# musyoku/chainer-speech-recognition

Measured on AMD Instinct MI355X. Metric: utterances/sec (T=1000, 40x3 feat, |V|~3000) CTC train step, higher is better.
Workload: dtype bf16

## Files before the change

### chainer-speech-recognition_amd/csrc/common.hpp

```cpp
#pragma once
#include <hip/hip_runtime.h>
#include <stdint.h>
#include <stddef.h>
#include <stdlib.h>
#include <string.h>

#define ASR_OK 0
#define ASR_ERR_BAD_ARG (-1)
#define ASR_ERR_WORKSPACE (-2)
#define ASR_ERR_UNSUPPORTED (-3)
#define ASR_ERR_LAUNCH (-4)

#define ASR_LAUNCH_CHECK()                                   \
    do {                                                     \
        if (hipGetLastError() != hipSuccess) return ASR_ERR_LAUNCH; \
    } while (0)

namespace asr {

constexpr int kWave = 64;

__device__ __forceinline__ float wave_sum(float v) {
#pragma unroll
    for (int o = 32; o > 0; o >>= 1) v += __shfl_xor(v, o, 64);
// ... 4 lines not shown
    for (int o = 32; o > 0; o >>= 1) v = fmaxf(v, __shfl_xor(v, o, 64));
    return v;
}
__device__ __forceinline__ double wave_sum_d(double v) {
#pragma unroll
    for (int o = 32; o > 0; o >>= 1) v += __shfl_xor(v, o, 64);
    return v;
}

__device__ __forceinline__ float block_sum(float v, float* scratch) {
    const int lane = threadIdx.x & 63, wid = threadIdx.x >> 6, nw = blockDim.x >> 6;
    v = wave_sum(v);
    if (lane == 0) scratch[wid] = v;
    __syncthreads();
    float r = 0.f;
    for (int i = 0; i < nw; ++i) r += scratch[i];
    __syncthreads();
    return r;
}
__device__ __forceinline__ float block_max(float v, float* scratch) {
    const int lane = threadIdx.x & 63, wid = threadIdx.x >> 6, nw = blockDim.x >> 6;
    v = wave_max(v);
    if (lane == 0) scratch[wid] = v;
    __syncthreads();
    float r = scratch[0];
    for (int i = 1; i < nw; ++i) r = fmaxf(r, scratch[i]);
    __syncthreads();
    return r;
}

#ifdef ASR_ACT_F16
#define ASR_ACT_IS_F16 1
__device__ __forceinline__ float bf16_to_f32(uint16_t h) {
    _Float16 v;
    __builtin_memcpy(&v, &h, 2);
    return (float)v;
}
__device__ __forceinline__ uint16_t f32_to_bf16(float f) {
    const _Float16 v = (_Float16)f;
    uint16_t h;
    __builtin_memcpy(&h, &v, 2);
    return h;
}
__device__ __forceinline__ uint32_t pack_bf16x2(float lo, float hi) {
    typedef _Float16 f16x2_t __attribute__((ext_vector_type(2)));
    typedef float f32x2_t __attribute__((ext_vector_type(2)));
    const f32x2_t v = {lo, hi};
    const f16x2_t r = __builtin_convertvector(v, f16x2_t);
    return *reinterpret_cast<const uint32_t*>(&r);
}
#define ASR_MFMA_16x16x32(a, b, c)                                                                                  \
    __builtin_amdgcn_mfma_f32_16x16x32_f16(__builtin_bit_cast(__attribute__((ext_vector_type(8))) _Float16, (a)),   \
                                           __builtin_bit_cast(__attribute__((ext_vector_type(8))) _Float16, (b)), (c), 0, 0, 0)
#else
#define ASR_ACT_IS_F16 0
__device__ __forceinline__ float bf16_to_f32(uint16_t h) { return __uint_as_float(((uint32_t)h) << 16); }
__device__ __forceinline__ uint16_t f32_to_bf16(float f) {
    __bf16 b = (__bf16)f;
    return *reinterpret_cast<uint16_t*>(&b);
}

__device__ __forceinline__ uint32_t pack_bf16x2(float lo, float hi) {
    typedef __bf16 bf16x2_t __attribute__((ext_vector_type(2)));
    typedef float f32x2_t __attribute__((ext_vector_type(2)));
    const f32x2_t v = {lo, hi};
    const bf16x2_t r = __builtin_convertvector(v, bf16x2_t);
    return *reinterpret_cast<const uint32_t*>(&r);
}
#define ASR_MFMA_16x16x32(a, b, c) __builtin_amdgcn_mfma_f32_16x16x32_bf16((a), (b), (c), 0, 0, 0)
#endif

static inline int debug_flag(const char* key, int dflt) {
    const char* e = getenv("ASR_DEBUG");
    if (!e) return dflt;
    const size_t n = strlen(key);
    for (const char* p = e; *p;) {
        while (*p == ',' || *p == ' ') ++p;
        if (strncmp(p, key, n) == 0 && p[n] == '=') return atoi(p + n + 1);
        while (*p && *p != ',') ++p;
    }
    return dflt;
}

static inline size_t align_up(size_t x, size_t a) { return (x + a - 1) / a * a; }
static inline int cdiv(long long a, long long b) { return (int)((a + b - 1) / b); }

}
```

### chainer-speech-recognition_amd/csrc/elementwise.hip

```cpp
#include "common.hpp"
#include "../../include/asr_hip.h"

namespace asr {
namespace ew {

constexpr int kThreads = 256;
static inline int grid_for(long long n) {
    long long g = (n + kThreads - 1) / kThreads;
    if (g > 256 * 16) g = 256 * 16;
    if (g < 1) g = 1;
    return (int)g;
}

__global__ void cast_bf16_kernel(const float* __restrict__ src, uint16_t* __restrict__ dst, long long n) {
    for (long long i = blockIdx.x * (long long)blockDim.x + threadIdx.x; i < n; i += (long long)gridDim.x * blockDim.x)
        dst[i] = f32_to_bf16(src[i]);
}
__global__ void cast_bf16_vec8_kernel(const float4* __restrict__ src, uint4* __restrict__ dst, long long n8) {
    for (long long i = blockIdx.x * (long long)blockDim.x + threadIdx.x; i < n8; i += (long long)gridDim.x * blockDim.x) {
        const float4 a = src[2 * i], b = src[2 * i + 1];
        uint4 o;
        o.x = (uint32_t)f32_to_bf16(a.x) | ((uint32_t)f32_to_bf16(a.y) << 16);
        o.y = (uint32_t)f32_to_bf16(a.z) | ((uint32_t)f32_to_bf16(a.w) << 16);
        o.z = (uint32_t)f32_to_bf16(b.x) | ((uint32_t)f32_to_bf16(b.y) << 16);
        o.w = (uint32_t)f32_to_bf16(b.z) | ((uint32_t)f32_to_bf16(b.w) << 16);
        dst[i] = o;
    }
}
__global__ void transpose_cast_kernel(const float* __restrict__ src, uint16_t* __restrict__ dst, int rows, int cols) {
    __shared__ float tile[32][33];
    const int r0 = blockIdx.y * 32, c0 = blockIdx.x * 32;
    const int tx = threadIdx.x & 31, ty = threadIdx.x >> 5;
    for (int i = ty; i < 32; i += 8) {
        const int r = r0 + i, c = c0 + tx;
        tile[i][tx] = (r < rows && c < cols) ? src[(size_t)r * cols + c] : 0.f;
    }
    __syncthreads();
    for (int i = ty; i < 32; i += 8) {
        const int c = c0 + i, r = r0 + tx;
        if (c < cols && r < rows) dst[(size_t)c * rows + r] = f32_to_bf16(tile[tx][i]);
    }
}
__global__ void __launch_bounds__(256) cast_many_kernel(const long long* __restrict__ jobs, int njobs) {
    __shared__ float tile[64][65];
    __shared__ long long first_tile[256];
    int j = 0;
    if (njobs <= 256) {
        if ((int)threadIdx.x < njobs) first_tile[threadIdx.x] = jobs[threadIdx.x * 6 + 5];
        __syncthreads();
        int lo = 0, hi = njobs - 1;
        while (lo < hi) {
            const int mid = (lo + hi + 1) >> 1;
            if (first_tile[mid] <= (long long)blockIdx.x) lo = mid; else hi = mid - 1;
        }
        j = lo;
    } else {
        while (j + 1 < njobs && (long long)blockIdx.x >= jobs[(j + 1) * 6 + 5]) ++j;
    }
    const float* __restrict__ src = (const float*)jobs[j * 6 + 0];
    uint16_t* __restrict__ dst = (uint16_t*)jobs[j * 6 + 1];
    const int rows = (int)jobs[j * 6 + 2], cols = (int)jobs[j * 6 + 3];
    const bool transpose = jobs[j * 6 + 4] != 0;
    const int local = (int)((long long)blockIdx.x - jobs[j * 6 + 5]);
    const int tiles_c = (cols + 63) / 64;
    const int r0 = (local / tiles_c) * 64, c0 = (local % tiles_c) * 64;
    const int tx = threadIdx.x & 15, ty = threadIdx.x >> 4;
    const bool vec = (cols & 3) == 0;
    if (!transpose) {
        for (int i = ty; i < 64; i += 16) {
            const int r = r0 + i, c = c0 + tx * 4;
            if (r >= rows || c >= cols) continue;
            if (vec) {
                const float4 v = *(const float4*)(src + (size_t)r * cols + c);
                uint2 o;
                o.x = (unsigned)f32_to_bf16(v.x) | ((unsigned)f32_to_bf16(v.y) << 16);
                o.y = (unsigned)f32_to_bf16(v.z) | ((unsigned)f32_to_bf16(v.w) << 16);
                *(uint2*)(dst + (size_t)r * cols + c) = o;
            } else {
                for (int k = 0; k < 4 && c + k < cols; ++k) dst[(size_t)r * cols + c + k] = f32_to_bf16(src[(size_t)r * cols + c + k]);
            }
        }
        return;
    }
    for (int i = ty; i < 64; i += 16) {
        const int r = r0 + i, c = c0 + tx * 4;
        if (vec && r < rows && c < cols) {
            const float4 v = *(const float4*)(src + (size_t)r * cols + c);
            tile[i][tx * 4 + 0] = v.x; tile[i][tx * 4 + 1] = v.y; tile[i][tx * 4 + 2] = v.z; tile[i][tx * 4 + 3] = v.w;
        } else {
            for (int k = 0; k < 4; ++k) tile[i][tx * 4 + k] = (r < rows && c + k < cols) ? src[(size_t)r * cols + c + k] : 0.f;
        }
    }
    __syncthreads();
    const bool vecr = (rows & 3) == 0;
    for (int i = ty; i < 64; i += 16) {
        const int c = c0 + i, r = r0 + tx * 4;
        if (c >= cols || r >= rows) continue;
        if (vecr) {
            uint2 o;
            o.x = (unsigned)f32_to_bf16(tile[tx * 4 + 0][i]) | ((unsigned)f32_to_bf16(tile[tx * 4 + 1][i]) << 16);
            o.y = (unsigned)f32_to_bf16(tile[tx * 4 + 2][i]) | ((unsigned)f32_to_bf16(tile[tx * 4 + 3][i]) << 16);
            *(uint2*)(dst + (size_t)c * rows + r) = o;
        } else {
            for (int k = 0; k < 4 && r + k < rows; ++k) dst[(size_t)c * rows + r + k] = f32_to_bf16(tile[tx * 4 + k][i]);
        }
    }
}
__global__ void bf16_to_f32_kernel(const uint16_t* __restrict__ src, float* __restrict__ dst, long long n) {
    for (long long i = blockIdx.x * (long long)blockDim.x + threadIdx.x; i < n; i += (long long)gridDim.x * blockDim.x)
        dst[i] = bf16_to_f32(src[i]);
}

template <typename SrcT, typename DstT>
__global__ void permute4_kernel(const SrcT* __restrict__ src, DstT* __restrict__ dst, int d0, int d1, int d2, int d3,
                                long long s0, long long s1, long long s2, long long s3) {
    const long long n = (long long)d0 * d1 * d2 * d3;
    for (long long i = blockIdx.x * (long long)blockDim.x + threadIdx.x; i < n; i += (long long)gridDim.x * blockDim.x) {
        long long r = i;
        const int i3 = r % d3; r /= d3;
        const int i2 = r % d2; r /= d2;
        const int i1 = r % d1; r /= d1;
        const int i0 = (int)r;
        const SrcT v = src[i0 * s0 + i1 * s1 + i2 * s2 + i3 * s3];
        float f;
        if (sizeof(SrcT) == 2) f = bf16_to_f32((uint16_t)v); else f = (float)v;
        if (sizeof(DstT) == 2) dst[i] = (DstT)f32_to_bf16(f); else dst[i] = (DstT)f;
    }
}

template <typename SrcT>
__global__ void pack_input_pad_kernel(const SrcT* __restrict__ x, long long sT, long long sB, long long sH, long long sC, int T,
                                      int B, int H, int C, int Cpad, uint16_t* __restrict__ out) {
    const long long n = (long long)T * B * H * Cpad;
    for (long long i = blockIdx.x * (long long)blockDim.x + threadIdx.x; i < n; i += (long long)gridDim.x * blockDim.x) {
        long long r = i;
        const int c = (int)(r % Cpad); r /= Cpad;
        const int h = (int)(r % H); r /= H;
        const int b = (int)(r % B);
        const int t = (int)(r / B);
        uint16_t v = 0;
        if (c < C) {
            const SrcT s = x[t * sT + b * sB + h * sH + c * sC];
            if (sizeof(SrcT) == 2) v = (uint16_t)s; else v = f32_to_bf16((float)s);
        }
        out[i] = v;
    }
}

constexpr int PIP = 72;
__global__ __launch_bounds__(256) void pack_input_pad_time_kernel(const float* __restrict__ x, long long sB, long long sH, long long sC,
                                                                 int T, int B, int H, int C, uint16_t* __restrict__ out) {
    __shared__ __attribute__((aligned(16))) uint16_t tile[64 * PIP];
    const int t0 = blockIdx.x * 64, b = blockIdx.y, h0 = blockIdx.z * 8;
    const int tl = threadIdx.x & 63, rg = threadIdx.x >> 6;
    for (int i = threadIdx.x; i < 64 * PIP / 2; i += 256) reinterpret_cast<uint32_t*>(tile)[i] = 0u;
    __syncthreads();
    for (int rr = rg; rr < C * 8; rr += 4) {
        const int c = rr >> 3, hh = rr & 7;
        if (h0 + hh < H && t0 + tl < T)
            tile[tl * PIP + hh * 8 + c] = f32_to_bf16(x[(long long)(t0 + tl) + b * sB + (h0 + hh) * sH + c * sC]);
    }
    __syncthreads();
#pragma unroll
    for (int k = 0; k < 2; ++k) {
        const int p = threadIdx.x + 256 * k, t = p >> 3, hh = p & 7;
        if (t0 + t < T && h0 + hh < H)
            *reinterpret_cast<uint4*>(out + (((long long)(t0 + t) * B + b) * H + h0 + hh) * 8) = *reinterpret_cast<const uint4*>(tile + t * PIP + hh * 8);
    }
}

template <typename SrcT>
__global__ void im2col_kernel(const SrcT* __restrict__ x, long long sT, long long sB, long long sH, long long sC, int T,
                              int B, int Hin, int Cin, int KH, int KW, int ph, int pt, int Tout, int Hout, int Kp,
                              uint16_t* __restrict__ col) {
    const long long rows = (long long)Tout * B * Hout;
    const long long n = rows * Kp;
    const int Kreal = KH * KW * Cin;
    for (long long i = blockIdx.x * (long long)blockDim.x + threadIdx.x; i < n; i += (long long)gridDim.x * blockDim.x) {
        const int k = (int)(i % Kp);
        long long row = i / Kp;
        uint16_t out = 0;
        if (k < Kreal) {
            const int ci = k % Cin;
            const int kw = (k / Cin) % KW;
            const int kh = k / (Cin * KW);
            const int ho = (int)(row % Hout); row /= Hout;
            const int b = (int)(row % B);
            const int t = (int)(row / B);
// ... 513 lines not shown
#pragma unroll
            for (int q = 0; q < RU; ++q) add(v[q]);
        }
        for (; r < r1; r += nrl) add(*reinterpret_cast<const uint4*>(x + r * ld + c8 * 8));
    }
    if (rl < nrl)
#pragma unroll
        for (int e = 0; e < 8; ++e) red[rl * cols + c8 * 8 + e] = acc[e];
    __syncthreads();
    for (int c = threadIdx.x; c < cols; c += blockDim.x) {
        float s2 = 0.f;
        for (int q = 0; q < nrl; ++q) s2 += red[q * cols + c];
        atomicAdd(out + c, s2);
    }
}

template <int NC>
__global__ __launch_bounds__(256) void colsum_wide_kernel(const uint16_t* __restrict__ x, long long rows, int cols, int ld,
                                                          float* __restrict__ out) {
    const int n8 = cols >> 3;
    const long long chunk = (rows + gridDim.x - 1) / gridDim.x;
    const long long r0 = blockIdx.x * chunk, r1 = min(rows, r0 + chunk);
    float acc[NC][8];
#pragma unroll
    for (int k = 0; k < NC; ++k)
#pragma unroll
        for (int e = 0; e < 8; ++e) acc[k][e] = 0.f;
    constexpr int RU = 4;
    for (long long r = r0; r < r1; r += RU) {
        uint4 v[RU][NC];
#pragma unroll
        for (int q = 0; q < RU; ++q)
#pragma unroll
            for (int k = 0; k < NC; ++k) {
                const int c8 = threadIdx.x + 256 * k;
                v[q][k] = (c8 < n8 && r + q < r1) ? *reinterpret_cast<const uint4*>(x + (r + q) * ld + c8 * 8) : make_uint4(0, 0, 0, 0);
            }
#pragma unroll
        for (int q = 0; q < RU; ++q)
#pragma unroll
            for (int k = 0; k < NC; ++k) {
                const uint32_t w[4] = {v[q][k].x, v[q][k].y, v[q][k].z, v[q][k].w};
#pragma unroll
                for (int e = 0; e < 4; ++e) {
                    acc[k][2 * e] += bf16_to_f32((uint16_t)(w[e] & 0xffff));
                    acc[k][2 * e + 1] += bf16_to_f32((uint16_t)(w[e] >> 16));
                }
            }
    }
#pragma unroll
    for (int k = 0; k < NC; ++k) {
        const int c8 = threadIdx.x + 256 * k;
        if (c8 < n8)
#pragma unroll
            for (int e = 0; e < 8; ++e) atomicAdd(out + c8 * 8 + e, acc[k][e]);
    }
}

}
}

using namespace asr;
using namespace asr::ew;

extern "C" int asr_cast_bf16(void* stream, const float* src, void* dst, int rows, int cols, int transpose) {
    if (!src || !dst || rows <= 0 || cols <= 0) return ASR_ERR_BAD_ARG;
    hipStream_t s = (hipStream_t)stream;
    if (!transpose) {
        const long long n = (long long)rows * cols;
        if ((n & 7) == 0 && ((((uintptr_t)src) | ((uintptr_t)dst)) & 15) == 0)
            hipLaunchKernelGGL(cast_bf16_vec8_kernel, dim3(grid_for(n >> 3)), dim3(kThreads), 0, s, (const float4*)src, (uint4*)dst, n >> 3);
        else
            hipLaunchKernelGGL(cast_bf16_kernel, dim3(grid_for(n)), dim3(kThreads), 0, s, src, (uint16_t*)dst, n);
    } else {
        hipLaunchKernelGGL(transpose_cast_kernel, dim3(cdiv(cols, 32), cdiv(rows, 32)), dim3(256), 0, s, src,
                           (uint16_t*)dst, rows, cols);
    }
    ASR_LAUNCH_CHECK();
    return ASR_OK;
}

extern "C" int asr_cast_bf16_many(void* stream, const long long* jobs_dev, int njobs, long long total_tiles) {
    if (!jobs_dev || njobs <= 0 || total_tiles <= 0 || total_tiles > 0x7fffffffLL) return ASR_ERR_BAD_ARG;
    hipLaunchKernelGGL(cast_many_kernel, dim3((unsigned)total_tiles), dim3(256), 0, (hipStream_t)stream, jobs_dev, njobs);
    ASR_LAUNCH_CHECK();
    return ASR_OK;
}

extern "C" int asr_bf16_to_f32(void* stream, const void* src, float* dst, long long n) {
    if (!src || !dst || n <= 0) return ASR_ERR_BAD_ARG;
    hipLaunchKernelGGL(bf16_to_f32_kernel, dim3(grid_for(n)), dim3(kThreads), 0, (hipStream_t)stream,
                       (const uint16_t*)src, dst, n);
    ASR_LAUNCH_CHECK();
    return ASR_OK;
}

extern "C" int asr_permute4(void* stream, const void* src, int src_bf16, void* dst, int dst_bf16, int d0, int d1, int d2,
                            int d3, long long s0, long long s1, long long s2, long long s3) {
    if (!src || !dst || d0 <= 0 || d1 <= 0 || d2 <= 0 || d3 <= 0) return ASR_ERR_BAD_ARG;
    hipStream_t s = (hipStream_t)stream;
    const long long n = (long long)d0 * d1 * d2 * d3;
    const dim3 g(grid_for(n)), b(kThreads);
    if (src_bf16 && dst_bf16)
        hipLaunchKernelGGL((permute4_kernel<uint16_t, uint16_t>), g, b, 0, s, (const uint16_t*)src, (uint16_t*)dst, d0, d1, d2, d3, s0, s1, s2, s3);
    else if (src_bf16)
        hipLaunchKernelGGL((permute4_kernel<uint16_t, float>), g, b, 0, s, (const uint16_t*)src, (float*)dst, d0, d1, d2, d3, s0, s1, s2, s3);
    else if (dst_bf16)
        hipLaunchKernelGGL((permute4_kernel<float, uint16_t>), g, b, 0, s, (const float*)src, (uint16_t*)dst, d0, d1, d2, d3, s0, s1, s2, s3);
    else
        hipLaunchKernelGGL((permute4_kernel<float, float>), g, b, 0, s, (const float*)src, (float*)dst, d0, d1, d2, d3, s0, s1, s2, s3);
    ASR_LAUNCH_CHECK();
    return ASR_OK;
}

extern "C" int asr_im2col(void* stream, const void* x, int x_bf16, long long sT, long long sB, long long sH, long long sC,
                          int T, int B, int Hin, int Cin, int KH, int KW, int pad_h, int pad_t, int Tout, int Kp,
                          void* col) {
    if (!x || !col || T <= 0 || B <= 0 || Hin <= 0 || Cin <= 0 || KH <= 0 || KW <= 0 || pad_h < 0 || pad_t < 0) return ASR_ERR_BAD_ARG;
    const int Hout = Hin + 2 * pad_h - KH + 1;
    if (Hout <= 0 || Kp < KH * KW * Cin || Tout <= 0 || Tout > T + 2 * pad_t - KW + 1) return ASR_ERR_BAD_ARG;
    const long long n = (long long)Tout * B * Hout * Kp;
    hipStream_t s = (hipStream_t)stream;
    if (x_bf16 && (Cin & 7) == 0 && (Kp & 7) == 0 && sC == 1 && sH == Cin && sB == (long long)Hin * Cin &&
        sT == (long long)B * Hin * Cin && ((((uintptr_t)x) | ((uintptr_t)col)) & 15) == 0 && Kp == KH * KW * Cin) {
        const long long nv = (long long)Tout * B * Hout * KH * KW * (Cin >> 3);
        hipLaunchKernelGGL(im2col_vec8_kernel, dim3(grid_for(nv)), dim3(kThreads), 0, s, (const uint16_t*)x, T, B, Hin, Cin, KH,
                           KW, pad_h, pad_t, Tout, Hout, Kp, (uint16_t*)col);
        ASR_LAUNCH_CHECK();
        return ASR_OK;
    }
    if ((Kp & 7) == 0 && (((uintptr_t)col) & 15) == 0) {
        const long long nc = n >> 3;
        if (x_bf16)
            hipLaunchKernelGGL(im2col_chunk8_kernel<uint16_t>, dim3(grid_for(nc)), dim3(kThreads), 0, s, (const uint16_t*)x, sT, sB, sH,
                               sC, T, B, Hin, Cin, KH, KW, pad_h, pad_t, Tout, Hout, Kp, (uint4*)col);
        else
            hipLaunchKernelGGL(im2col_chunk8_kernel<float>, dim3(grid_for(nc)), dim3(kThreads), 0, s, (const float*)x, sT, sB, sH, sC,
                               T, B, Hin, Cin, KH, KW, pad_h, pad_t, Tout, Hout, Kp, (uint4*)col);
        ASR_LAUNCH_CHECK();
        return ASR_OK;
    }
    if (x_bf16)
        hipLaunchKernelGGL(im2col_kernel<uint16_t>, dim3(grid_for(n)), dim3(kThreads), 0, s, (const uint16_t*)x, sT, sB, sH,
                           sC, T, B, Hin, Cin, KH, KW, pad_h, pad_t, Tout, Hout, Kp, (uint16_t*)col);
    else
        hipLaunchKernelGGL(im2col_kernel<float>, dim3(grid_for(n)), dim3(kThreads), 0, s, (const float*)x, sT, sB, sH, sC,
                           T, B, Hin, Cin, KH, KW, pad_h, pad_t, Tout, Hout, Kp, (uint16_t*)col);
    ASR_LAUNCH_CHECK();
    return ASR_OK;
}

extern "C" int asr_col2im(void* stream, const void* dcol, int T, int B, int Hin, int Cin, int KH, int KW, int pad_h,
                          int pad_t, int Tout, int Kp, void* dx) {
    if (!dcol || !dx || T <= 0 || B <= 0 || Hin <= 0 || Cin <= 0 || pad_h < 0 || pad_t < 0) return ASR_ERR_BAD_ARG;
    const int Hout = Hin + 2 * pad_h - KH + 1;
    if (Hout <= 0 || Kp < KH * KW * Cin || Tout <= 0 || Tout > T + 2 * pad_t - KW + 1) return ASR_ERR_BAD_ARG;
    const long long n = (long long)T * B * Hin * Cin;
    if ((Cin & 7) == 0 && (Kp & 7) == 0 && ((((uintptr_t)dcol) | ((uintptr_t)dx)) & 15) == 0) {
        hipLaunchKernelGGL(col2im_vec8_kernel, dim3(grid_for(n >> 3)), dim3(kThreads), 0, (hipStream_t)stream,
                           (const uint16_t*)dcol, T, B, Hin, Cin, KH, KW, pad_h, pad_t, Tout, Hout, Kp, (uint16_t*)dx);
        ASR_LAUNCH_CHECK();
        return ASR_OK;
    }
    hipLaunchKernelGGL(col2im_kernel, dim3(grid_for(n)), dim3(kThreads), 0, (hipStream_t)stream, (const uint16_t*)dcol, T,
                       B, Hin, Cin, KH, KW, pad_h, pad_t, Tout, Hout, Kp, (uint16_t*)dx);
    ASR_LAUNCH_CHECK();
    return ASR_OK;
// ... 211 lines not shown
```

### chainer-speech-recognition_amd/csrc/layernorm.hip

```cpp
#include "common.hpp"
#include "../../include/asr_hip.h"

namespace asr {
namespace ln {

template <typename T>
__device__ __forceinline__ float ldf(const T* p, long long i) {
    if (sizeof(T) == 2) return bf16_to_f32((uint16_t)p[i]);
    return (float)p[i];
}
template <typename T>
__device__ __forceinline__ void stf(T* p, long long i, float v) {
    if (sizeof(T) == 2) p[i] = (T)f32_to_bf16(v); else p[i] = (T)v;
}

__device__ __forceinline__ float usable_rstd(float r) { return r < INFINITY ? r : 0.f; }

template <typename XT, typename YT>
__global__ __launch_bounds__(256) void fwd_kernel(const XT* __restrict__ x, YT* __restrict__ y,
                                                  const float* __restrict__ gamma, const float* __restrict__ beta,
                                                  float* __restrict__ mean_out, float* __restrict__ rstd_out, int D,
                                                  int C) {
    __shared__ float scratch[32];
    const long long row = blockIdx.x;
// ... 298 lines not shown
        else atomicAdd(extra + (col - 2 * D), total);
    }
}


template <int MODE>
__global__ __launch_bounds__(256) void bn_reduce_kernel(const uint16_t* __restrict__ x, const uint16_t* __restrict__ gy,
                                                        const float* __restrict__ mean, const float* __restrict__ rstd,
                                                        long long R, int C, int rows_per_block, double* __restrict__ out0,
                                                        double* __restrict__ out1) {
    const long long r0 = (long long)blockIdx.x * rows_per_block;
    const long long r1 = r0 + rows_per_block < R ? r0 + rows_per_block : R;
    for (int c = threadIdx.x; c < C; c += blockDim.x) {
        float a = 0.f, b = 0.f;
        const float mu = MODE ? mean[c] : 0.f, rs = MODE ? rstd[c] : 0.f;
        for (long long r = r0; r < r1; ++r) {
            const float xv = bf16_to_f32(x[r * C + c]);
            if (MODE == 0) { a += xv; b += xv * xv; }
            else { const float g = bf16_to_f32(gy[r * C + c]); a += g; b += g * (xv - mu) * rs; }
        }
        atomicAdd(out0 + c, (double)a);
        atomicAdd(out1 + c, (double)b);
    }
}

__global__ void bn_finish_kernel(const double* __restrict__ s, const double* __restrict__ q, long long R, int C, float eps,
                                 float decay, float* __restrict__ mean, float* __restrict__ rstd, float* __restrict__ avg_mean,
                                 float* __restrict__ avg_var) {
    const int c = blockIdx.x * blockDim.x + threadIdx.x;
    if (c >= C) return;
    const double mu = s[c] / (double)R;
    double var = q[c] / (double)R - mu * mu;
    if (var < 0.0) var = 0.0;
    mean[c] = (float)mu;
    rstd[c] = (float)(1.0 / sqrt(var + (double)eps));
    if (avg_mean) {
        const double unbiased = R > 1 ? var * (double)R / (double)(R - 1) : var;
        avg_mean[c] = decay * avg_mean[c] + (1.f - decay) * (float)mu;
        avg_var[c] = decay * avg_var[c] + (1.f - decay) * (float)unbiased;
    }
}

__global__ void bn_fwd_kernel(const uint16_t* __restrict__ x, const float* __restrict__ mean, const float* __restrict__ rstd,
                              const float* __restrict__ gamma, const float* __restrict__ beta, long long n, int C,
                              uint16_t* __restrict__ y) {
    for (long long i = blockIdx.x * (long long)blockDim.x + threadIdx.x; i < n; i += (long long)gridDim.x * blockDim.x) {
        const int c = (int)(i % C);
        y[i] = f32_to_bf16(gamma[c] * (bf16_to_f32(x[i]) - mean[c]) * rstd[c] + beta[c]);
    }
}

__global__ void bn_bwd_kernel(const uint16_t* __restrict__ x, const uint16_t* __restrict__ gy, const float* __restrict__ mean,
                              const float* __restrict__ rstd, const float* __restrict__ gamma, const double* __restrict__ sgy,
                              const double* __restrict__ sgx, long long R, int C, uint16_t* __restrict__ dx) {
    const long long n = R * C;
    for (long long i = blockIdx.x * (long long)blockDim.x + threadIdx.x; i < n; i += (long long)gridDim.x * blockDim.x) {
        const int c = (int)(i % C);
        const float xhat = (bf16_to_f32(x[i]) - mean[c]) * rstd[c];
        const float a = (float)(sgy[c] / (double)R), b = (float)(sgx[c] / (double)R);
        dx[i] = f32_to_bf16(gamma[c] * rstd[c] * (bf16_to_f32(gy[i]) - a - xhat * b));
    }
}

__global__ void bn_param_grad_kernel(const double* __restrict__ sgy, const double* __restrict__ sgx, int C,
                                     float* __restrict__ dgamma, float* __restrict__ dbeta) {
    const int c = blockIdx.x * blockDim.x + threadIdx.x;
    if (c >= C) return;
    atomicAdd(dgamma + c, (float)sgx[c]);
    atomicAdd(dbeta + c, (float)sgy[c]);
}

}
}

using namespace asr;
using namespace asr::ln;

static bool fwd_rows_ok(const void* x, const void* y, const float* gamma, const float* beta, int D, int C) {
    return C == D && (D & 3) == 0 && D <= 4096 && ((((uintptr_t)x) | ((uintptr_t)y) | ((uintptr_t)gamma) | ((uintptr_t)beta)) & 15) == 0;
}
static int launch_fwd_rows(hipStream_t s, const float* x, float* y, const float* gamma, const float* beta, float* mean, float* rstd,
                           float* lse, long long rows, int D) {
    long long blocks = (rows + 3) / 4;
    if (blocks > 256 * 3) blocks = 256 * 3;
    const int nv = cdiv(D >> 2, 64);
#define ASR_LNF(NV) hipLaunchKernelGGL(fwd_rows_f32_kernel<NV>, dim3((unsigned)blocks), dim3(256), 0, s, x, y, gamma, beta, mean, rstd, lse, rows, D)
    if (nv <= 4) ASR_LNF(4); else if (nv <= 8) ASR_LNF(8); else if (nv <= 12) ASR_LNF(12); else ASR_LNF(16);
#undef ASR_LNF
    ASR_LAUNCH_CHECK();
    return ASR_OK;
}

extern "C" int asr_layernorm_fwd_lse_ok(int D, int C) { return C == D && (D & 3) == 0 && D <= 4096; }

extern "C" int asr_layernorm_fwd_lse(void* stream, const float* x, float* y, const float* gamma, const float* beta, float* mean,
                                     float* rstd, float* lse, long long rows, int D) {
    if (!x || !y || !gamma || !beta || !mean || !rstd || rows <= 0 || D <= 0) return ASR_ERR_BAD_ARG;
    if (!fwd_rows_ok(x, y, gamma, beta, D, D)) return ASR_ERR_UNSUPPORTED;
    return launch_fwd_rows((hipStream_t)stream, x, y, gamma, beta, mean, rstd, lse, rows, D);
}

extern "C" int asr_layernorm_fwd(void* stream, const void* x, int x_bf16, void* y, int y_bf16, const float* gamma,
                                 const float* beta, float* mean, float* rstd, long long rows, int D, int C) {
    if (!x || !y || !gamma || !beta || !mean || !rstd || rows <= 0 || D <= 0 || C <= 0 || D % C) return ASR_ERR_BAD_ARG;
    hipStream_t s = (hipStream_t)stream;
    if (!x_bf16 && !y_bf16 && fwd_rows_ok(x, y, gamma, beta, D, C))
        return launch_fwd_rows(s, (const float*)x, (float*)y, gamma, beta, mean, rstd, nullptr, rows, D);
    const dim3 g((unsigned)rows), b(256);
    if (!x_bf16 && !y_bf16 && (D & 3) == 0 && (C & 3) == 0 && ((((uintptr_t)x) | ((uintptr_t)y)) & 15) == 0) {
        hipLaunchKernelGGL(fwd_f32x4_kernel, g, b, 0, s, (const float*)x, (float*)y, gamma, beta, mean, rstd, D, C);
        ASR_LAUNCH_CHECK();
        return ASR_OK;
    }
    if (x_bf16 && y_bf16)
        hipLaunchKernelGGL((fwd_kernel<uint16_t, uint16_t>), g, b, 0, s, (const uint16_t*)x, (uint16_t*)y, gamma, beta, mean, rstd, D, C);
    else if (x_bf16)
        hipLaunchKernelGGL((fwd_kernel<uint16_t, float>), g, b, 0, s, (const uint16_t*)x, (float*)y, gamma, beta, mean, rstd, D, C);
    else if (y_bf16)
        hipLaunchKernelGGL((fwd_kernel<float, uint16_t>), g, b, 0, s, (const float*)x, (uint16_t*)y, gamma, beta, mean, rstd, D, C);
    else
        hipLaunchKernelGGL((fwd_kernel<float, float>), g, b, 0, s, (const float*)x, (float*)y, gamma, beta, mean, rstd, D, C);
    ASR_LAUNCH_CHECK();
    return ASR_OK;
}

template <typename XT, typename GT>
static int launch_bwd(hipStream_t s, const void* x, const void* dy, const float* gamma, const float* mean,
                      const float* rstd, void* dx, int dx_bf16, float* dgamma, float* dbeta, long long rows, int D,
                      int C) {
    const dim3 g((unsigned)rows), b(256);
    if (dx && sizeof(XT) == 4 && sizeof(GT) == 4 && !dx_bf16 && (D & 3) == 0 && (C & 3) == 0 &&
        ((((uintptr_t)x) | ((uintptr_t)dy) | ((uintptr_t)dx)) & 15) == 0) {
        hipLaunchKernelGGL(bwd_f32x4_kernel, g, b, 0, s, (const float*)x, (const float*)dy, gamma, mean, rstd, (float*)dx, D, C);
        ASR_LAUNCH_CHECK();
    } else if (dx) {
        if (dx_bf16)
            hipLaunchKernelGGL((bwd_kernel<XT, GT, uint16_t>), g, b, 0, s, (const XT*)x, (const GT*)dy, gamma, mean, rstd, (uint16_t*)dx, D, C);
        else
            hipLaunchKernelGGL((bwd_kernel<XT, GT, float>), g, b, 0, s, (const XT*)x, (const GT*)dy, gamma, mean, rstd, (float*)dx, D, C);
        ASR_LAUNCH_CHECK();
    }
    if (dgamma && dbeta) {
        int chunks = (int)((rows + 127) / 128);
        if (chunks > 64) chunks = 64;
        hipLaunchKernelGGL((param_grad_kernel<XT, GT>), dim3(cdiv(D, 64), chunks), dim3(256), 0, s, (const XT*)x,
                           (const GT*)dy, mean, rstd, rows, D, C, dgamma, dbeta);
        ASR_LAUNCH_CHECK();
    }
    return ASR_OK;
}

extern "C" int asr_layernorm_bwd(void* stream, const void* x, int x_bf16, const void* dy, int dy_bf16,
                                 const float* gamma, const float* mean, const float* rstd, void* dx, int dx_bf16,
                                 float* dgamma, float* dbeta, long long rows, int D, int C) {
    if (!x || !dy || !gamma || !mean || !rstd || rows <= 0 || D <= 0 || C <= 0 || D % C) return ASR_ERR_BAD_ARG;
    hipStream_t s = (hipStream_t)stream;
    if (x_bf16 && dy_bf16) return launch_bwd<uint16_t, uint16_t>(s, x, dy, gamma, mean, rstd, dx, dx_bf16, dgamma, dbeta, rows, D, C);
    if (x_bf16) return launch_bwd<uint16_t, float>(s, x, dy, gamma, mean, rstd, dx, dx_bf16, dgamma, dbeta, rows, D, C);
    if (dy_bf16) return launch_bwd<float, uint16_t>(s, x, dy, gamma, mean, rstd, dx, dx_bf16, dgamma, dbeta, rows, D, C);
    return launch_bwd<float, float>(s, x, dy, gamma, mean, rstd, dx, dx_bf16, dgamma, dbeta, rows, D, C);
}

static int rows_grid(long long rows) {
    long long g = (rows + 15) / 16;
    if (g > 1024) g = 1024;
    if (g < 1) g = 1;
    return (int)g;
// ... 212 lines not shown
```

Before: 2475.

## Make batched bf16 cast persistent with prefetch, size grids by CU count

The multi-tensor fp32-to-bf16 cast kernel becomes a persistent grid-stride loop sized to a multiple of the device CU count. Each block caches the whole job table in LDS and software-prefetches the next tile's loads before storing the current one. Non-transposed jobs are now handled as flat 4096-element chunks with 16-byte vector loads and stores instead of 64x64 row tiles. The LayerNorm forward row kernel's grid cap also switches from a fixed constant to a CU-count multiple. The aim is to cut block launch and scheduling overhead and hide load latency, at the cost of more complex tile-walk logic and a job-table layout that must match the host's tile counting for flat chunks.

```diff
diff --git a/chainer-speech-recognition_amd/csrc/common.hpp b/chainer-speech-recognition_amd/csrc/common.hpp
--- a/chainer-speech-recognition_amd/csrc/common.hpp
+++ b/chainer-speech-recognition_amd/csrc/common.hpp
@@ -110,6 +110,18 @@
     return dflt;
 }
 
+static inline int device_cu_count() {
+    static int cached[64];
+    int dev = 0;
+    if (hipGetDevice(&dev) != hipSuccess || dev < 0 || dev >= 64) return 256;
+    if (cached[dev] == 0) {
+        int n = 0;
+        if (hipDeviceGetAttribute(&n, hipDeviceAttributeMultiprocessorCount, dev) != hipSuccess) n = 0;
+        cached[dev] = n > 0 ? n : 256;
+    }
+    return cached[dev];
+}
+
 static inline size_t align_up(size_t x, size_t a) { return (x + a - 1) / a * a; }
 static inline int cdiv(long long a, long long b) { return (int)((a + b - 1) / b); }
 
diff --git a/chainer-speech-recognition_amd/csrc/elementwise.hip b/chainer-speech-recognition_amd/csrc/elementwise.hip
--- a/chainer-speech-recognition_amd/csrc/elementwise.hip
+++ b/chainer-speech-recognition_amd/csrc/elementwise.hip
@@ -41,69 +41,177 @@
         if (c < cols && r < rows) dst[(size_t)c * rows + r] = f32_to_bf16(tile[tx][i]);
     }
 }
-__global__ void __launch_bounds__(256) cast_many_kernel(const long long* __restrict__ jobs, int njobs) {
+#define CM_GLOBAL __attribute__((address_space(1)))
+typedef float cm_f32x4 __attribute__((ext_vector_type(4)));
+typedef uint32_t cm_u32x4 __attribute__((ext_vector_type(4)));
+typedef uint32_t cm_u32x2 __attribute__((ext_vector_type(2)));
+struct CastTile {
+    const CM_GLOBAL float* src;
+    CM_GLOBAL uint16_t* dst;
+    int transpose;
+    int vec_ld, vec_st;
+    long long n, e0;
+    int rows, cols, r0, c0;
+    long long resume;
+};
+constexpr int kCastManyLds = 256;
+constexpr int kCastChunk = 4096;
+
+template <bool IN_LDS>
+__device__ __forceinline__ long long cm_entry(const long long* __restrict__ jobs, const long long* tab, int i) {
+    return IN_LDS ? tab[i] : jobs[i];
+}
+template <bool IN_LDS>
+__device__ __forceinline__ CastTile cm_describe(const long long* __restrict__ jobs, const long long* tab, int njobs, long long total_tiles,
+                                                long long t, int& j) {
+    int lo = j, hi = njobs - 1;
+    while (lo < hi) {
+        const int mid = (lo + hi + 1) >> 1;
+        if (cm_entry<IN_LDS>(jobs, tab, mid * 6 + 5) <= t) lo = mid; else hi = mid - 1;
+    }
+    j = lo;
+    CastTile d;
+    d.src = (const CM_GLOBAL float*)cm_entry<IN_LDS>(jobs, tab, j * 6 + 0);
+    d.dst = (CM_GLOBAL uint16_t*)cm_entry<IN_LDS>(jobs, tab, j * 6 + 1);
+    d.rows = (int)cm_entry<IN_LDS>(jobs, tab, j * 6 + 2);
+    d.cols = (int)cm_entry<IN_LDS>(jobs, tab, j * 6 + 3);
+    d.transpose = cm_entry<IN_LDS>(jobs, tab, j * 6 + 4) != 0;
+    const long long local = t - cm_entry<IN_LDS>(jobs, tab, j * 6 + 5);
+    const bool src16 = (((uintptr_t)d.src) & 15) == 0;
+    d.resume = 0;
+    d.n = (long long)d.rows * d.cols;
+    d.e0 = local * kCastChunk;
+    d.r0 = d.c0 = 0;
+    if (d.transpose) {
+        const int tiles_c = (d.cols + 63) / 64;
+        d.r0 = (int)(local / tiles_c) * 64;
+        d.c0 = (int)(local % tiles_c) * 64;
+        d.vec_ld = (d.cols & 3) == 0 && src16;
+        d.vec_st = (d.rows & 3) == 0 && (((uintptr_t)d.dst) & 7) == 0;
+    } else {
+        d.vec_ld = d.vec_st = src16 && (((uintptr_t)d.dst) & 15) == 0;
+        if (d.e0 >= d.n) d.resume = j + 1 < njobs ? cm_entry<IN_LDS>(jobs, tab, (j + 1) * 6 + 5) : total_tiles;
+    }
+    return d;
+}
+__device__ __forceinline__ float4 cm_load4(const CM_GLOBAL float* p) {
+    const cm_f32x4 t = *(const CM_GLOBAL cm_f32x4*)p;
+    return make_float4(t.x, t.y, t.z, t.w);
+}
+__device__ __forceinline__ float cm_load1(const CM_GLOBAL float* p, bool in) {
+    float v = 0.f;
+    if (in) v = *p;
+    return v;
+}
+__device__ __forceinline__ void cm_load(const CastTile& d, float4 (&v)[4]) {
+    if (!d.transpose) {
+#pragma unroll
+        for (int p = 0; p < 2; ++p) {
+            const long long e = d.e0 + p * (kCastChunk / 2) + threadIdx.x * 8;
+            const CM_GLOBAL float* s = d.src + e;
+            if (d.vec_ld && e + 8 <= d.n) {
+                v[2 * p] = cm_load4(s);
+                v[2 * p + 1] = cm_load4(s + 4);
+            } else {
+                v[2 * p] = make_float4(cm_load1(s + 0, e + 0 < d.n), cm_load1(s + 1, e + 1 < d.n), cm_load1(s + 2, e + 2 < d.n), cm_load1(s + 3, e + 3 < d.n));
+                v[2 * p + 1] = make_float4(cm_load1(s + 4, e + 4 < d.n), cm_load1(s + 5, e + 5 < d.n), cm_load1(s + 6, e + 6 < d.n), cm_load1(s + 7, e + 7 < d.n));
+            }
+        }
+        return;
+    }
+    const int tx = threadIdx.x & 15, ty = threadIdx.x >> 4;
+#pragma unroll
+    for (int q = 0; q < 4; ++q) {
+        const int r = d.r0 + ty + 16 * q, c = d.c0 + tx * 4;
+        const CM_GLOBAL float* s = d.src + (size_t)r * d.cols + c;
+        const bool in = r < d.rows;
+        if (d.vec_ld) {
+            v[q] = make_float4(0.f, 0.f, 0.f, 0.f);
+            if (in && c < d.cols) v[q] = cm_load4(s);
+        } else {
+            v[q] = make_float4(cm_load1(s + 0, in && c + 0 < d.cols), cm_load1(s + 1, in && c + 1 < d.cols), cm_load1(s + 2, in && c + 2 < d.cols),
+                               cm_load1(s + 3, in && c + 3 < d.cols));
+        }
+    }
+}
+__device__ __forceinline__ uint32_t cm_pack(float lo, float hi) { return (unsigned)f32_to_bf16(lo) | ((unsigned)f32_to_bf16(hi) << 16); }
+__device__ __forceinline__ void cm_store(const CastTile& d, const float4 (&v)[4], float (*tile)[65]) {
+    if (!d.transpose) {
+#pragma unroll
+        for (int p = 0; p < 2; ++p) {
+            const long long e = d.e0 + p * (kCastChunk / 2) + threadIdx.x * 8;
+            CM_GLOBAL uint16_t* o = d.dst + e;
+            const float4 a = v[2 * p], b = v[2 * p + 1];
+            if (d.vec_st && e + 8 <= d.n) {
+                *(CM_GLOBAL cm_u32x4*)o = cm_u32x4{cm_pack(a.x, a.y), cm_pack(a.z, a.w), cm_pack(b.x, b.y), cm_pack(b.z, b.w)};
+            } else {
+                const float f[8] = {a.x, a.y, a.z, a.w, b.x, b.y, b.z, b.w};
+#pragma unroll
+                for (int k = 0; k < 8; ++k)
+                    if (e + k < d.n) o[k] = f32_to_bf16(f[k]);
+            }
+        }
+        return;
+    }
+    const int tx = threadIdx.x & 15, ty = threadIdx.x >> 4;
+#pragma unroll
+    for (int q = 0; q < 4; ++q) {
+        const int i = ty + 16 * q;
+        tile[i][tx * 4 + 0] = v[q].x; tile[i][tx * 4 + 1] = v[q].y; tile[i][tx * 4 + 2] = v[q].z; tile[i][tx * 4 + 3] = v[q].w;
+    }
+    __syncthreads();
+#pragma unroll
+    for (int q = 0; q < 4; ++q) {
+        const int i = ty + 16 * q, c = d.c0 + i, r = d.r0 + tx * 4;
+        if (c >= d.cols || r >= d.rows) continue;
+        CM_GLOBAL uint16_t* o = d.dst + (size_t)c * d.rows + r;
+        if (d.vec_st) {
+            *(CM_GLOBAL cm_u32x2*)o = cm_u32x2{cm_pack(tile[tx * 4 + 0][i], tile[tx * 4 + 1][i]), cm_pack(tile[tx * 4 + 2][i], tile[tx * 4 + 3][i])};
+        } else {
+            for (int k = 0; k < 4 && r + k < d.rows; ++k) o[k] = f32_to_bf16(tile[tx * 4 + k][i]);
+        }
+    }
+    __syncthreads();
+}
+template <bool IN_LDS>
+__device__ __forceinline__ long long cm_seek(const long long* __restrict__ jobs, const long long* tab, int njobs, long long total_tiles,
+                                             long long t, int& j, CastTile& d) {
+    while (t < total_tiles) {
+        d = cm_describe<IN_LDS>(jobs, tab, njobs, total_tiles, t, j);
+        if (d.resume <= t) break;
+        t += (d.resume - t + gridDim.x - 1) / gridDim.x * gridDim.x;
+    }
+    return t;
+}
+template <bool IN_LDS>
+__device__ __forceinline__ void cm_walk(const long long* __restrict__ jobs, const long long* tab, int njobs, long long total_tiles,
+                                        float (*tile)[65]) {
+    int j = 0;
+    CastTile cur, nxt;
+    long long t = cm_seek<IN_LDS>(jobs, tab, njobs, total_tiles, blockIdx.x, j, cur);
+    if (t >= total_tiles) return;
+    float4 v[4], vn[4];
+    cm_load(cur, v);
+    for (;;) {
+        t = cm_seek<IN_LDS>(jobs, tab, njobs, total_tiles, t + gridDim.x, j, nxt);
+        const bool more = t < total_tiles;
+        if (more) cm_load(nxt, vn);
+        cm_store(cur, v, tile);
+        if (!more) break;
+        cur = nxt;
+#pragma unroll
+        for (int q = 0; q < 4; ++q) v[q] = vn[q];
+    }
+}
+__global__ void __launch_bounds__(256) cast_many_kernel(const long long* __restrict__ jobs, int njobs, long long total_tiles) {
     __shared__ float tile[64][65];
-    __shared__ long long first_tile[256];
-    int j = 0;
-    if (njobs <= 256) {
-        if ((int)threadIdx.x < njobs) first_tile[threadIdx.x] = jobs[threadIdx.x * 6 + 5];
+    __shared__ long long tab[kCastManyLds * 6];
+    if (njobs <= kCastManyLds) {
+        for (int i = threadIdx.x; i < njobs * 6; i += 256) tab[i] = jobs[i];
         __syncthreads();
-        int lo = 0, hi = njobs - 1;
-        while (lo < hi) {
-            const int mid = (lo + hi + 1) >> 1;
-            if (first_tile[mid] <= (long long)blockIdx.x) lo = mid; else hi = mid - 1;
-        }
-        j = lo;
+        cm_walk<true>(jobs, tab, njobs, total_tiles, tile);
     } else {
-        while (j + 1 < njobs && (long long)blockIdx.x >= jobs[(j + 1) * 6 + 5]) ++j;
-    }
-    const float* __restrict__ src = (const float*)jobs[j * 6 + 0];
-    uint16_t* __restrict__ dst = (uint16_t*)jobs[j * 6 + 1];
-    const int rows = (int)jobs[j * 6 + 2], cols = (int)jobs[j * 6 + 3];
-    const bool transpose = jobs[j * 6 + 4] != 0;
-    const int local = (int)((long long)blockIdx.x - jobs[j * 6 + 5]);
-    const int tiles_c = (cols + 63) / 64;
-    const int r0 = (local / tiles_c) * 64, c0 = (local % tiles_c) * 64;
-    const int tx = threadIdx.x & 15, ty = threadIdx.x >> 4;
-    const bool vec = (cols & 3) == 0;
-    if (!transpose) {
-        for (int i = ty; i < 64; i += 16) {
-            const int r = r0 + i, c = c0 + tx * 4;
-            if (r >= rows || c >= cols) continue;
-            if (vec) {
-                const float4 v = *(const float4*)(src + (size_t)r * cols + c);
-                uint2 o;
-                o.x = (unsigned)f32_to_bf16(v.x) | ((unsigned)f32_to_bf16(v.y) << 16);
-                o.y = (unsigned)f32_to_bf16(v.z) | ((unsigned)f32_to_bf16(v.w) << 16);
-                *(uint2*)(dst + (size_t)r * cols + c) = o;
-            } else {
-                for (int k = 0; k < 4 && c + k < cols; ++k) dst[(size_t)r * cols + c + k] = f32_to_bf16(src[(size_t)r * cols + c + k]);
-            }
-        }
-        return;
-    }
-    for (int i = ty; i < 64; i += 16) {
-        const int r = r0 + i, c = c0 + tx * 4;
-        if (vec && r < rows && c < cols) {
-            const float4 v = *(const float4*)(src + (size_t)r * cols + c);
-            tile[i][tx * 4 + 0] = v.x; tile[i][tx * 4 + 1] = v.y; tile[i][tx * 4 + 2] = v.z; tile[i][tx * 4 + 3] = v.w;
-        } else {
-            for (int k = 0; k < 4; ++k) tile[i][tx * 4 + k] = (r < rows && c + k < cols) ? src[(size_t)r * cols + c + k] : 0.f;
-        }
-    }
-    __syncthreads();
-    const bool vecr = (rows & 3) == 0;
-    for (int i = ty; i < 64; i += 16) {
-        const int c = c0 + i, r = r0 + tx * 4;
-        if (c >= cols || r >= rows) continue;
-        if (vecr) {
-            uint2 o;
-            o.x = (unsigned)f32_to_bf16(tile[tx * 4 + 0][i]) | ((unsigned)f32_to_bf16(tile[tx * 4 + 1][i]) << 16);
-            o.y = (unsigned)f32_to_bf16(tile[tx * 4 + 2][i]) | ((unsigned)f32_to_bf16(tile[tx * 4 + 3][i]) << 16);
-            *(uint2*)(dst + (size_t)c * rows + r) = o;
-        } else {
-            for (int k = 0; k < 4 && r + k < rows; ++k) dst[(size_t)c * rows + r + k] = f32_to_bf16(tile[tx * 4 + k][i]);
-        }
+        cm_walk<false>(jobs, tab, njobs, total_tiles, tile);
     }
 }
 __global__ void bf16_to_f32_kernel(const uint16_t* __restrict__ src, float* __restrict__ dst, long long n) {
@@ -783,7 +891,9 @@
 
 extern "C" int asr_cast_bf16_many(void* stream, const long long* jobs_dev, int njobs, long long total_tiles) {
     if (!jobs_dev || njobs <= 0 || total_tiles <= 0 || total_tiles > 0x7fffffffLL) return ASR_ERR_BAD_ARG;
-    hipLaunchKernelGGL(cast_many_kernel, dim3((unsigned)total_tiles), dim3(256), 0, (hipStream_t)stream, jobs_dev, njobs);
+    long long grid = (long long)device_cu_count() * 5;
+    if (grid > total_tiles) grid = total_tiles;
+    hipLaunchKernelGGL(cast_many_kernel, dim3((unsigned)grid), dim3(256), 0, (hipStream_t)stream, jobs_dev, njobs, total_tiles);
     ASR_LAUNCH_CHECK();
     return ASR_OK;
 }
diff --git a/chainer-speech-recognition_amd/csrc/layernorm.hip b/chainer-speech-recognition_amd/csrc/layernorm.hip
--- a/chainer-speech-recognition_amd/csrc/layernorm.hip
+++ b/chainer-speech-recognition_amd/csrc/layernorm.hip
@@ -404,7 +404,8 @@
 static int launch_fwd_rows(hipStream_t s, const float* x, float* y, const float* gamma, const float* beta, float* mean, float* rstd,
                            float* lse, long long rows, int D) {
     long long blocks = (rows + 3) / 4;
-    if (blocks > 256 * 3) blocks = 256 * 3;
+    const long long cap = (long long)device_cu_count() * 8;
+    if (blocks > cap) blocks = cap;
     const int nv = cdiv(D >> 2, 64);
 #define ASR_LNF(NV) hipLaunchKernelGGL(fwd_rows_f32_kernel<NV>, dim3((unsigned)blocks), dim3(256), 0, s, x, y, gamma, beta, mean, rstd, lse, rows, D)
     if (nv <= 4) ASR_LNF(4); else if (nv <= 8) ASR_LNF(8); else if (nv <= 12) ASR_LNF(12); else ASR_LNF(16);
```

Result: no change. 2480 (median of 6 runs) (+0.2%).
